# Peter00796/dlrover_wuqiong

Measured on AMD Instinct MI355X. Metric: ckpt save/load sec GPT2-1.5B; goodput% under injected faults at 1/2/4/8 GPU, lower is better.
Workload: dtype bf16

## Files before the change

dlrover_wuqiong_amd/_native/kernel_sigs.py:

```python

import ctypes as c

vp, i64, i32, u32, u64, f32, cp = (c.c_void_p, c.c_int64, c.c_int, c.c_uint32, c.c_uint64,
                                   c.c_float, c.c_char_p)

SIGS = {
    "dw_fp8_cast_amax": (i32, [vp, i32, vp, vp, vp, i64, i32, vp]),
    "dw_fp8_update_scales": (i32, [vp, vp, vp, vp, vp, i32, i32, i32, f32, vp]),
    "dw_fp8_cast_t": (i32, [vp, i32, vp, vp, vp, vp, i32, i32, i32, vp]),
    "dw_multi_copy": (i32, [vp, i64, vp]),
    "dw_gemm_dgelu": (i32, [vp, vp, vp, vp, i32, i32, i32, vp]),
    "dw_gemm_dgelu_bgrad": (i32, [vp, vp, vp, vp, vp, i32, i32, i32, vp]),
    "dw_gemm_wgrad_bgradb": (i32, [vp, vp, vp, vp, i32, i32, i32, i32, vp]),
    "dw_multi_copy_grid": (i32, [vp, i64, i32, vp]),
    "dw_multi_copy_variant": (i32, [vp, i64, i32, i32, vp]),
    "dw_fill_u32": (i32, [vp, i64, u32, vp]),
    "dw_host_register": (i32, [vp, u64]),
    "dw_host_unregister": (i32, [vp]),
    "dw_host_registered": (i32, [vp]),
    "dw_memcpy_async": (i32, [vp, vp, u64, i32, vp]),
    "dw_stream_sync": (i32, [vp]),
    "dw_event_sync": (i32, [vp]),
    "dw_stream_create_cumask": (vp, [i32, c.POINTER(i32)]),
    "dw_stream_destroy": (i32, [vp]),
# ... 39 lines not shown
    "dw_norm_fwd": (i32, [vp, vp, vp, vp, vp, vp, i64, i32, f32, i32, vp]),
    "dw_bias_gelu_fwd": (i32, [vp, vp, vp, vp, i64, i32, vp]),
    "dw_gelu_bwd": (i32, [vp, vp, vp, i64, vp]),
    "dw_colsum_parts": (i32, [i64]),
    "dw_colsum": (i32, [vp, i64, i32, vp, vp, i32, vp]),
    "dw_qadamw": (i32, [vp, vp, vp, vp, vp, vp, i64, i64, i32, i32, i32, f32, f32, f32, f32, f32, f32, f32, f32,
                        vp]),
    "dw_qadam_flat": (i32, [vp, i32, vp, vp, i32, vp, vp, vp, vp, vp, i64, i64, f32, f32, f32, f32, f32, f32, f32,
                            i32, vp, i32, vp]),
    "dw_colsum_acc": (i32, [vp, i64, i32, vp, vp, i32, i32, vp, vp]),
    "dw_gelu_bwd_dbias": (i32, [vp, vp, vp, i64, i32, vp, vp, i32, i32, vp, vp]),
    "dw_norm_bwd": (i32, [vp, vp, vp, vp, vp, vp, vp, vp, vp, vp, vp, i64, i64, i32, i32, i32, i32, vp, vp, vp]),
    "dw_norm_bwd_part_floats": (i64, [i64, i32, i32]),
    "dw_colred_det_floats": (i64, [i64, i32, i32]),
    "dw_add_norm_fwd": (i32, [vp, vp, vp, vp, vp, vp, vp, vp, i64, i32, f32, i32, vp]),
    "dw_swiglu_fwd": (i32, [vp, vp, i64, i32, vp]),
    "dw_swiglu_bwd": (i32, [vp, vp, vp, i64, i32, vp]),
    "dw_rope": (i32, [vp, vp, vp, vp, i64, i32, i32, i32, i32, vp, i32, vp]),
    "dw_qkv_rope": (i32, [vp, vp, vp, vp, vp, vp, i64, i32, i32, i32, i32, i32, vp, i32, vp]),
    "dw_grouped_gemm": (i32, [i32, vp, vp, vp, vp, i32, i32, i32, i32, i32, c.c_longlong, c.c_longlong,
                              c.c_longlong, c.c_longlong, c.c_longlong, vp]),
    "dw_grouped_glu_fwd": (i32, [vp, vp, vp, vp, vp, vp, i32, i32, i32, i32, vp]),
    "dw_grouped_glu_dgrad": (i32, [vp, vp, vp, vp, vp, i32, i32, i32, i32, vp]),
    "dw_xent_fwd": (i32, [vp, vp, vp, vp, vp, vp, i64, i32, i64, i64, f32, vp]),
    "dw_xent_bwd": (i32, [vp, vp, vp, vp, i32, vp, i64, i32, i64, i64, f32, vp]),
    "dw_token_logprob_fwd": (i32, [vp, i32, vp, vp, vp, vp, i64, i64, i64, i64, i32, vp]),
    "dw_token_logprob_bwd": (i32, [vp, i32, vp, vp, vp, vp, vp, vp, i64, i64, i64, i64, i32, vp]),
    "dw_sample_tokens": (i32, [vp, i32, vp, vp, i32, i32, i64, f32, i32, f32, u64, vp]),
    "dw_kv_append_rope": (i32, [vp, vp, vp, vp, vp, vp, vp, i64, i32, i32, i32, i32, i32, i64, i64, i32, vp]),
    "dw_rollout_step": (i32, [vp, vp, vp, vp, vp, vp, vp, i32, i64, i64, i64, vp]),
    "dw_moe_route_ws_floats": (i64, [i64]),
    "dw_moe_route_fwd": (i32, [vp, i32, vp, vp, vp, vp, vp, vp, vp, i64, i32, i32, i32, f32, f32, vp]),
    "dw_moe_route_bwd": (i32, [vp, i32, vp, vp, vp, vp, vp, vp, vp, i64, i32, i32, i32, f32, f32, vp]),
    "dw_moe_sort_ws_size": (i64, [i64, i32]),
    "dw_moe_sort_chunk_size": (i32, []),
    "dw_moe_sort": (i32, [vp, i64, i32, vp, vp, vp, vp, vp]),
    "dw_moe_gather_rows": (i32, [vp, vp, vp, vp, vp, vp, vp, i32, i64, i64, i32, i32, vp]),
    "dw_moe_ksum_rows": (i32, [vp, vp, vp, vp, vp, i32, i64, i64, i32, i32, vp]),
}

class AttnExtArgs(c.Structure):

    _fields_ = [("bias_bs", i64), ("bias_hs", i64), ("bias_qs", i64), ("bias", vp), ("prefix", vp), ("seed", u64),
                ("offset", u64), ("win_l", i32), ("win_r", i32), ("p_drop", f32), ("pad_", i32), ("alibi", vp),
                ("alibi_bs", i64)]


class AttnCall(c.Structure):

    _fields_ = [("q", vp), ("k", vp), ("v", vp), ("o", vp), ("lse", vp), ("dout", vp), ("dq", vp), ("dk", vp),
                ("dv", vp), ("workspace", vp), ("strides", i64 * 16), ("cu_q", vp), ("cu_k", vp),
                ("ext", AttnExtArgs), ("stream", vp), ("B", i32), ("Sq", i32), ("Sk", i32), ("H", i32),
                ("HKV", i32), ("D", i32), ("total_q", i32), ("total_k", i32), ("causal", i32), ("variant", i32),
                ("softmax_scale", f32), ("pad_", i32)]


OPTIONAL = {
    "dw_attn_fwd": (i32, [c.POINTER(AttnCall)]),
    "dw_attn_bwd": (i32, [c.POINTER(AttnCall)]),
    "dw_attn_bwd_workspace": (i64, [i32, i32, i32, i32]),
    "dw_attn_call_size": (i32, []),
    "dw_attn_dropout_mask": (i32, [vp, i32, i32, i32, f32, u64, u64, vp]),
    "dw_attn_decode": (i32, [vp, vp, vp, vp, vp, vp, vp, i32, i32, i32, i32, i32, i32, vp, f32, vp]),
    "dw_moe_regroup": (i32, [vp, vp, vp, i32, i32, i64, i32, i32, vp]),
}


def declare(lib):
    for name, (res, args) in SIGS.items():
        f = getattr(lib, name)
        f.restype = res
        f.argtypes = args
    for name, (res, args) in OPTIONAL.items():
        f = getattr(lib, name, None)
        if f is not None:
            f.restype = res
            f.argtypes = args
    size = getattr(lib, "dw_attn_call_size", None)
    if size is not None and size() != c.sizeof(AttnCall):
        raise RuntimeError(f"AttnCall ABI mismatch: library {size()} bytes, ctypes mirror {c.sizeof(AttnCall)}")
```

dlrover_wuqiong_amd/csrc/kernels/attn_bwd.hip:

```cpp
#include "attn_common.h"

#include <cstdlib>

typedef __attribute__((ext_vector_type(4))) short s16x4;
typedef __attribute__((address_space(3))) s16x4 lds_s16x4;
#define LDS_PTR(p) ((__attribute__((address_space(3))) void*)(p))

__device__ __forceinline__ bf16x8_t as_bf(const u32x4& v) { return __builtin_bit_cast(bf16x8_t, v); }

__device__ __forceinline__ unsigned int pk2(float a, float b) {
  typedef __bf16 bf16x2_v __attribute__((ext_vector_type(2)));
  typedef float f32x2_v __attribute__((ext_vector_type(2)));
  return __builtin_bit_cast(unsigned int, __builtin_convertvector((f32x2_v){a, b}, bf16x2_v));
}

__device__ __forceinline__ u32x4 scaled8(const u32x4& v, float c) {
  float f[8];
  unpack8(v, f);
  return (u32x4){pk2(f[0] * c, f[1] * c), pk2(f[2] * c, f[3] * c), pk2(f[4] * c, f[5] * c), pk2(f[6] * c, f[7] * c)};
}

template <int D>
__device__ __forceinline__ u32x4 tr_frag(const char* img, int r0, int d0, const int (&tr)[2]) {
  const s16x4 v0 =
      __builtin_amdgcn_ds_read_tr16_b64_v4i16((lds_s16x4*)LDS_PTR(img + tr[0] + tr_const<D>(r0, d0 / 32, 0)));
  const s16x4 v1 =
      __builtin_amdgcn_ds_read_tr16_b64_v4i16((lds_s16x4*)LDS_PTR(img + tr[1] + tr_const<D>(r0, d0 / 32, 1)));
  return join_tr(v0, v1);
}

template <int D>
__global__ void __launch_bounds__(256) attn_bwd_pre_kernel(const bf16_t* __restrict__ O, const bf16_t* __restrict__ dO,
                                                           float* __restrict__ delta, int B, int S, int H,
                                                           AttnStrides st) {
  constexpr int LPR = D / 8;
  constexpr int RPW = 64 / LPR;
  const int lane = threadIdx.x & 63;
  const int64_t row = ((int64_t)blockIdx.x * 4 + (threadIdx.x >> 6)) * RPW + lane / LPR;
  const int c = lane % LPR;
  const bool ok = row < (int64_t)B * S * H;
  float acc = 0.f;
  int h = 0, s = 0, b = 0;
  if (ok) {
    h = (int)(row % H);
    const int64_t bs = row / H;
    s = (int)(bs % S);
    b = (int)(bs / S);
    float a[8], d[8];
    unpack8(*(const u32x4*)(O + (int64_t)b * st.o_bs + (int64_t)s * st.o_rs + h * D + c * 8), a);
    unpack8(*(const u32x4*)(dO + (int64_t)b * st.do_bs + (int64_t)s * st.do_rs + h * D + c * 8), d);
#pragma unroll
    for (int k = 0; k < 8; ++k) acc += a[k] * d[k];
  }
#pragma unroll
  for (int off = LPR / 2; off > 0; off >>= 1) acc += __shfl_xor(acc, off, 64);
  if (ok && c == 0) delta[((int64_t)b * H + h) * S + s] = acc;
}


template <int D>
struct DkvCfg {
  static constexpr int WAVES = 4;
  static constexpr int BKB = 32 * WAVES;
  static constexpr int BQT = D == 64 ? 64 : 32;
  static constexpr int NCH = D / 8;
  static constexpr int KK = D / 16;
  static constexpr int DT = D / 32;
  static constexpr int TILE = BQT * D * 2;
  static constexpr int BUF = 2 * TILE + 2 * BQT * 4;
  static constexpr int VPT = BQT * NCH / (64 * WAVES);
  static constexpr int VIMG = BKB * D * 2;
};

template <int D, bool CAUSAL, bool PARTIAL, bool EXT>
__global__ void __launch_bounds__(64 * DkvCfg<D>::WAVES, (D == 64 && !EXT) ? 3 : 2)
attn_bwd_dkdv_kernel(const bf16_t* __restrict__ Q, const bf16_t* __restrict__ K, const bf16_t* __restrict__ V,
                     const bf16_t* __restrict__ dO, const float* __restrict__ LSE, const float* __restrict__ DELTA,
                     bf16_t* __restrict__ dK, bf16_t* __restrict__ dV, float* __restrict__ dKp,
                     float* __restrict__ dVp, int S, int H, int HKV, float scale, float scale_log2,
                     AttnStrides st, AttnVarlen vl, AttnExt ex) {
  using C = DkvCfg<D>;
  extern __shared__ __attribute__((aligned(16))) char smem[];
  const int tid = threadIdx.x, lane = tid & 63;
  const int wid = __builtin_amdgcn_readfirstlane(tid >> 6);
  const int r = lane & 31, hh = lane >> 5;
  const BlockXYZ bc = xcd_block((S + C::BKB - 1) / C::BKB, H);
  const int b = bc.z, h = bc.y;
  const int hk = h / (H / HKV);
  const int kb0 = bc.x * C::BKB;
  const SeqRange sr = seq_range(vl, b, h, H, S);
  if (kb0 >= sr.sk) return;
  const int SQ = sr.sq, SK = sr.sk, co = SK - SQ;
  const int kw0 = kb0 + 32 * wid;
  const int key = kw0 + r;
  const bf16_t* Qb = Q + (int64_t)b * st.q_bs + (int64_t)sr.q_off * st.q_rs + (int64_t)h * D;
  const bf16_t* dOb = dO + (int64_t)b * st.do_bs + (int64_t)sr.q_off * st.do_rs + (int64_t)h * D;
  const bf16_t* Kb = K + (int64_t)b * st.k_bs + (int64_t)sr.k_off * st.k_rs + (int64_t)hk * D;
  const bf16_t* Vb = V + (int64_t)b * st.v_bs + (int64_t)sr.k_off * st.v_rs + (int64_t)hk * D;
  const float* lse_b = LSE + sr.lse_base;
  const float* del_b = DELTA + sr.lse_base;

  char* v_img = smem + 2 * C::BUF;
  constexpr bool VDMA = !EXT && (C::VIMG / 1024) % C::WAVES == 0;
  if constexpr (VDMA) {
    constexpr int NGV = C::VIMG / 1024 / C::WAVES;
#pragma unroll
    for (int j = 0; j < NGV; ++j) {
      const int ci = NGV * wid + j;
      int row, ch;
      dma_rc<D>(ci, lane, row, ch);
      const int kv = min(kb0 + row, SK - 1);
      __builtin_amdgcn_global_load_lds((const void*)(Vb + (int64_t)kv * st.v_rs + ch * 8),
                                       LDS_PTR(v_img + 1024 * ci), 16, 0, 0);
    }
  }
  for (int v = tid; v < (VDMA ? 0 : C::BKB * C::NCH); v += 64 * C::WAVES) {
    int row, c;
    stage_rc<D>(v, row, c);
    const int kv = kb0 + row;
    *(u32x4*)(v_img + img_off<D>(row, c)) =
        kv < SK ? *(const u32x4*)(Vb + (int64_t)kv * st.v_rs + c * 8) : (u32x4){0, 0, 0, 0};
  }
  u32x4 kf[C::KK];
#pragma unroll
  for (int kk = 0; kk < C::KK; ++kk)
    kf[kk] = key < SK ? scaled8(*(const u32x4*)(Kb + (int64_t)key * st.k_rs + 16 * kk + 8 * hh), scale_log2)
                      : (u32x4){0, 0, 0, 0};
  f32x16 dk[C::DT], dv[C::DT];
#pragma unroll
  for (int dt = 0; dt < C::DT; ++dt)
#pragma unroll
    for (int i = 0; i < 16; ++i) {
      dk[dt][i] = 0.f;
// ... 144 lines not shown
          for (int j = 0; j < 4; ++j) {
            const int i = 4 * g + j;
            {
              const int q = q0 + qi + j;
              const bool vis = (q < SQ) && ext_visible(ex, CAUSAL, q, key, co, SK, pre);
              float add = (vis && ex.bias)
                  ? ex.bias[(int64_t)b * ex.bias_bs + (int64_t)h * ex.bias_hs + (int64_t)q * ex.bias_qs + key] *
                        1.4426950408889634f
                  : 0.f;
              add -= al2 * fabsf((float)(key - q - co));
              const float p = vis ? __builtin_amdgcn_exp2f(s[i] + add) : 0.f;
              if (ex.dropout) {
                const float del = -stl[C::BQT + qi + j];
                const bool kp = attn_keep(ex, bh, (long long)sr.q_off + q, (long long)sr.k_off + key);
                s[i] = kp ? p * ex.inv_keep : 0.f;
                dp[i] = p * (kp ? (dp[i] + del) * ex.inv_keep - del : -del);
              } else {
                s[i] = p;
                dp[i] = p * dp[i];
              }
            }
          }
        }
#pragma unroll
        for (int s2 = 0; s2 < 2; ++s2) {
          const u32x4 pf = {pk2(s[8 * s2 + 0], s[8 * s2 + 1]), pk2(s[8 * s2 + 2], s[8 * s2 + 3]),
                            pk2(s[8 * s2 + 4], s[8 * s2 + 5]), pk2(s[8 * s2 + 6], s[8 * s2 + 7])};
          const u32x4 sf = {pk2(dp[8 * s2 + 0], dp[8 * s2 + 1]), pk2(dp[8 * s2 + 2], dp[8 * s2 + 3]),
                            pk2(dp[8 * s2 + 4], dp[8 * s2 + 5]), pk2(dp[8 * s2 + 6], dp[8 * s2 + 7])};
#pragma unroll
          for (int dt = 0; dt < C::DT; ++dt) {
            const u32x4 doT = tr_frag<D>(dl, 32 * qs + 16 * s2, 32 * dt, trl);
            dv[dt] = __builtin_amdgcn_mfma_f32_32x32x16_bf16(as_bf(doT), as_bf(pf), dv[dt], 0, 0, 0);
          }
#pragma unroll
          for (int dt = 0; dt < C::DT; ++dt) {
            const u32x4 qT = tr_frag<D>(ql, 32 * qs + 16 * s2, 32 * dt, trl);
            dk[dt] = __builtin_amdgcn_mfma_f32_32x32x16_bf16(as_bf(qT), as_bf(sf), dk[dt], 0, 0, 0);
          }
        }
      }
    }
    if (it + 1 < n_it) {
      write((it + 1) & 1);
      if (!DMA && it + 2 < n_it) issue(it + 2);
    }
    if constexpr (DMA) asm volatile("s_waitcnt vmcnt(0)" ::: "memory");
    __syncthreads();
    if (DMA && it + 2 < n_it) {
      dma(it + 2, it & 1);
      issue(it + 2);
    }
  }
  if (key >= SK) return;
  if (PARTIAL) {
    const int64_t prow = vl.cu_q ? (int64_t)sr.k_off + key : (int64_t)b * S + key;
    float* kp = dKp + (prow * H + h) * D;
    float* vp = dVp + (prow * H + h) * D;
#pragma unroll
    for (int dt = 0; dt < C::DT; ++dt)
#pragma unroll
      for (int g = 0; g < 4; ++g) {
        const int d = 32 * dt + 8 * g + 4 * hh;
        *(f32x4*)(kp + d) = (f32x4){dk[dt][4 * g] * scale, dk[dt][4 * g + 1] * scale, dk[dt][4 * g + 2] * scale,
                                    dk[dt][4 * g + 3] * scale};
        *(f32x4*)(vp + d) = (f32x4){dv[dt][4 * g], dv[dt][4 * g + 1], dv[dt][4 * g + 2], dv[dt][4 * g + 3]};
      }
  } else {
    bf16_t* dKk = dK + (int64_t)b * st.dk_bs + (int64_t)hk * D + (int64_t)(sr.k_off + key) * st.dk_rs;
    bf16_t* dVk = dV + (int64_t)b * st.dv_bs + (int64_t)hk * D + (int64_t)(sr.k_off + key) * st.dv_rs;
#pragma unroll
    for (int dt = 0; dt < C::DT; ++dt)
#pragma unroll
      for (int g = 0; g < 4; ++g) {
        const int d = 32 * dt + 8 * g + 4 * hh;
        uint2 wk, wv;
        wk.x = pk2(dk[dt][4 * g] * scale, dk[dt][4 * g + 1] * scale);
        wk.y = pk2(dk[dt][4 * g + 2] * scale, dk[dt][4 * g + 3] * scale);
        wv.x = pk2(dv[dt][4 * g], dv[dt][4 * g + 1]);
        wv.y = pk2(dv[dt][4 * g + 2], dv[dt][4 * g + 3]);
        *(uint2*)(dKk + d) = wk;
        *(uint2*)(dVk + d) = wv;
      }
  }
}

template <int D>
__global__ void gqa_reduce_kernel(const float* __restrict__ pk, const float* __restrict__ pv, bf16_t* __restrict__ dK,
                                  bf16_t* __restrict__ dV, int64_t BS, int S, int H, int HKV, AttnStrides st) {
  const int group = H / HKV;
  const int64_t nv = BS * HKV * (D / 8);
  for (int64_t i = blockIdx.x * (int64_t)blockDim.x + threadIdx.x; i < nv; i += (int64_t)gridDim.x * blockDim.x) {
    const int c = (int)(i % (D / 8));
    const int64_t t = i / (D / 8);
    const int hk = (int)(t % HKV);
    const int64_t bs = t / HKV;
    const int64_t b = bs / S, sq = bs % S;
    float fk[8] = {0, 0, 0, 0, 0, 0, 0, 0}, fv[8] = {0, 0, 0, 0, 0, 0, 0, 0};
    for (int g = 0; g < group; ++g) {
      const int64_t off = (bs * H + hk * group + g) * D + c * 8;
      const f32x4 a0 = *(const f32x4*)(pk + off), a1 = *(const f32x4*)(pk + off + 4);
      const f32x4 b0 = *(const f32x4*)(pv + off), b1 = *(const f32x4*)(pv + off + 4);
#pragma unroll
      for (int j = 0; j < 4; ++j) {
        fk[j] += a0[j];
        fk[4 + j] += a1[j];
        fv[j] += b0[j];
        fv[4 + j] += b1[j];
      }
    }
    *(u32x4*)(dK + b * st.dk_bs + sq * st.dk_rs + hk * D + c * 8) = pack8(fk);
    *(u32x4*)(dV + b * st.dv_bs + sq * st.dv_rs + hk * D + c * 8) = pack8(fv);
  }
}

template <int D>
struct DqCfg {
  static constexpr int WAVES = D == 64 ? 4 : 8;
  static constexpr int BQ = 32 * WAVES;
  static constexpr int BK = 64;
  static constexpr int NCH = D / 8;
  static constexpr int KK = D / 16;
  static constexpr int DT = D / 32;
  static constexpr int TILE = BK * D * 2;
  static constexpr int VPT = BK * NCH / (64 * WAVES);
};

template <int D, bool CAUSAL, bool EXT>
__global__ void __launch_bounds__(64 * DqCfg<D>::WAVES, (D == 64 && !EXT) ? 3 : 1)
attn_bwd_dq_kernel(const bf16_t* __restrict__ Q, const bf16_t* __restrict__ K, const bf16_t* __restrict__ V,
                   const bf16_t* __restrict__ dO, const float* __restrict__ LSE, const float* __restrict__ DELTA,
                   bf16_t* __restrict__ dQ, int S, int H, int HKV, float scale, float scale_log2, AttnStrides st,
                   AttnVarlen vl, AttnExt ex) {
  using C = DqCfg<D>;
  extern __shared__ __attribute__((aligned(16))) char smem[];
  const int tid = threadIdx.x, lane = tid & 63;
  const int wid = __builtin_amdgcn_readfirstlane(tid >> 6);
  const int r = lane & 31, hh = lane >> 5;
  const int nqb = (S + C::BQ - 1) / C::BQ;
  const BlockXYZ bc = xcd_block(nqb, H);
  const int b = bc.z, h = bc.y;
  const int hk = h / (H / HKV);
  const int qblk = CAUSAL ? nqb - 1 - bc.x : bc.x;
  const int q_blk0 = qblk * C::BQ;
  const SeqRange sr = seq_range(vl, b, h, H, S);
  if (q_blk0 >= sr.sq) return;
  const int SQ = sr.sq, SK = sr.sk, co = SK - SQ;
  const int q0 = q_blk0 + wid * 32;
  const int q = q0 + r;
  const bf16_t* Qb = Q + (int64_t)b * st.q_bs + (int64_t)sr.q_off * st.q_rs + (int64_t)h * D;
  const bf16_t* dOb = dO + (int64_t)b * st.do_bs + (int64_t)sr.q_off * st.do_rs + (int64_t)h * D;
  const bf16_t* Kb = K + (int64_t)b * st.k_bs + (int64_t)sr.k_off * st.k_rs + (int64_t)hk * D;
  const bf16_t* Vb = V + (int64_t)b * st.v_bs + (int64_t)sr.k_off * st.v_rs + (int64_t)hk * D;

  constexpr bool RI = !EXT && D == 128;
  u32x4 qf[C::KK], dof[C::KK];
#pragma unroll
  for (int kk = 0; kk < C::KK; ++kk) {
    if (q < SQ) {
      qf[kk] = *(const u32x4*)(Qb + (int64_t)q * st.q_rs + 16 * kk + 8 * hh);
      if (RI) qf[kk] = scaled8(qf[kk], scale_log2);
      dof[kk] = *(const u32x4*)(dOb + (int64_t)q * st.do_rs + 16 * kk + 8 * hh);
    } else {
      qf[kk] = (u32x4){0, 0, 0, 0};
      dof[kk] = (u32x4){0, 0, 0, 0};
    }
  }
  const int64_t so = sr.lse_base + q;
  const float lse_v = q < SQ ? LSE[so] : -INFINITY;
  const float lse2 = lse_v > -INFINITY ? lse_v * 1.4426950408889634f : INFINITY;
  const float dl = q < SQ ? DELTA[so] : 0.f;

  f32x16 acc[C::DT];
#pragma unroll
  for (int dt = 0; dt < C::DT; ++dt)
#pragma unroll
    for (int i = 0; i < 16; ++i) acc[dt][i] = 0.f;
  constexpr bool DPI = !EXT && D == 64;
  f32x16 s_init, dp_init;
#pragma unroll
  for (int i = 0; i < 16; ++i) {
    s_init[i] = -lse2;
    dp_init[i] = -dl;
  }

  int n_tiles = (SK + C::BK - 1) / C::BK;
// ... 111 lines not shown
        if (!EXT) {
          if (need_mask) {
            __asm__ volatile("");
            const int rel = lim - k0 - 32 * sb - 4 * hh;
#pragma unroll
            for (int i = 0; i < 16; ++i) s[i] = ((i & 3) + 8 * (i >> 2)) < rel ? s[i] : -INFINITY;
          }
#pragma unroll
          for (int i = 0; i < 16; ++i) {
            if (RI) {
              s[i] = __builtin_amdgcn_exp2f(s[i]) * dp[i];
            } else {
              const float p = __builtin_amdgcn_exp2f(__builtin_fmaf(s[i], scale_log2, -lse2));
              s[i] = p * (DPI ? dp[i] : dp[i] - dl);
            }
          }
        }
#pragma unroll
        for (int i = 0; i < 16 && EXT; ++i) {
          {
            const int key = k0 + 32 * sb + (i & 3) + 8 * (i >> 2) + 4 * hh;
            const bool vis = (q < SQ) && ext_visible(ex, CAUSAL, q, key, co, SK, pre);
            float add = (vis && brow) ? brow[key] * 1.4426950408889634f : 0.f;
            add -= al2 * fabsf((float)(key - q - co));
            const float p = vis ? __builtin_amdgcn_exp2f(__builtin_fmaf(s[i], scale_log2, add - lse2)) : 0.f;
            float dpe = dp[i];
            if (ex.dropout)
              dpe = attn_keep(ex, bh, (long long)sr.q_off + q, (long long)sr.k_off + key) ? dpe * ex.inv_keep : 0.f;
            s[i] = p * (dpe - dl);
          }
        }
#pragma unroll
        for (int s2 = 0; s2 < 2; ++s2) {
          const u32x4 pf = {pk2(s[8 * s2 + 0], s[8 * s2 + 1]), pk2(s[8 * s2 + 2], s[8 * s2 + 3]),
                            pk2(s[8 * s2 + 4], s[8 * s2 + 5]), pk2(s[8 * s2 + 6], s[8 * s2 + 7])};
#pragma unroll
          for (int dt = 0; dt < C::DT; ++dt) {
            const u32x4 kt = tr_frag<D>(kl, 32 * sb + 16 * s2, 32 * dt, trl);
            acc[dt] = __builtin_amdgcn_mfma_f32_32x32x16_bf16(as_bf(kt), as_bf(pf), acc[dt], 0, 0, 0);
          }
        }
      }
      };
      tile();
    }
    if (!DMA && tt + 1 < n_run) {
      write_lds((tt + 1) & 1);
      if (tt + 2 < n_run) issue_load(t + 2);
    }
    if constexpr (DMA) asm volatile("s_waitcnt vmcnt(0)" ::: "memory");
    __syncthreads();
    if (DMA && tt + 2 < n_run) dma(t + 2, tt & 1);
  }
  if (q < SQ) {
    bf16_t* dQq = dQ + (int64_t)b * st.dq_bs + (int64_t)h * D + (int64_t)(sr.q_off + q) * st.dq_rs;
#pragma unroll
    for (int dt = 0; dt < C::DT; ++dt)
#pragma unroll
      for (int g = 0; g < 4; ++g) {
        uint2 w;
        w.x = pk2(acc[dt][4 * g + 0] * scale, acc[dt][4 * g + 1] * scale);
        w.y = pk2(acc[dt][4 * g + 2] * scale, acc[dt][4 * g + 3] * scale);
        *(uint2*)(dQq + 32 * dt + 8 * g + 4 * hh) = w;
      }
  }
}

extern "C" int64_t dw_attn_bwd_workspace(int B, int S, int H, int D) {
  return (int64_t)B * H * S * 4 + 2 * (int64_t)B * S * H * D * 4 + 512;
}

struct SideStream {
  hipStream_t s = nullptr;
  hipEvent_t fork = nullptr, join = nullptr;
};

static SideStream* side_stream() {
  static thread_local SideStream per_dev[16];
  int d = 0;
  if (hipGetDevice(&d) != hipSuccess || d < 0 || d >= 16) return nullptr;
  SideStream& ss = per_dev[d];
  if (!ss.s) {
    if (hipStreamCreateWithFlags(&ss.s, hipStreamNonBlocking) != hipSuccess) return nullptr;
    if (hipEventCreateWithFlags(&ss.fork, hipEventDisableTiming) != hipSuccess ||
        hipEventCreateWithFlags(&ss.join, hipEventDisableTiming) != hipSuccess)
      return nullptr;
  }
  return &ss;
}

static bool bwd_concurrent() {
  static const bool on = [] {
    const char* v = getenv("DWAMD_ATTN_BWD_CONCURRENT");
    return !(v && v[0] == '0');
  }();
  return on;
}

template <int D>
static void launch_bwd(const AttnCall& c, const AttnVarlen& vl, const AttnExt* ext) {
  const AttnExt none = {};
  const AttnExt& ex = ext ? *ext : none;
  const AttnStrides& st = c.st;
  const int B = c.B, Sq = c.Sq, Sk = c.Sk, H = c.H, HKV = c.HKV;
  const bool causal = c.causal;
  hipStream_t s = (hipStream_t)c.stream;
  char* ws = (char*)c.workspace;
  const bf16_t *q = (const bf16_t*)c.q, *k = (const bf16_t*)c.k, *v = (const bf16_t*)c.v;
  const bf16_t* dout = (const bf16_t*)c.dout;
  const float* lse = (const float*)c.lse;
  const int Smax = Sq > Sk ? Sq : Sk;
  float* delta = (float*)ws;
  const int pre_b = vl.cu_q ? 1 : B, pre_s = vl.cu_q ? vl.total_q : Sq;
  const int64_t rows = (int64_t)pre_b * pre_s * H;
  constexpr int RPB = 4 * (64 / (D / 8));
  hipLaunchKernelGGL(attn_bwd_pre_kernel<D>, dim3((unsigned)((rows + RPB - 1) / RPB)), dim3(256), 0, s,
                     (const bf16_t*)c.o, dout, delta, pre_b, pre_s, H, st);
  const float scale_log2 = c.softmax_scale * 1.4426950408889634f;
  SideStream* side = bwd_concurrent() ? side_stream() : nullptr;
  hipStream_t sq = s;
  if (side && hipEventRecord(side->fork, s) == hipSuccess && hipStreamWaitEvent(side->s, side->fork, 0) == hipSuccess)
    sq = side->s;
  using KC = DkvCfg<D>;
  const bool partial = H != HKV;
  float* pk = (float*)(ws + (((int64_t)B * H * Smax * 4 + 255) / 256) * 256);
  float* pv = pk + (int64_t)B * Smax * H * D;
  dim3 gk((unsigned)((Sk + KC::BKB - 1) / KC::BKB * H * B));
  const int lk = 2 * KC::BUF + KC::VIMG;
#define DKDV(CA, PA, EX)                                                                                    \
  hipLaunchKernelGGL((attn_bwd_dkdv_kernel<D, CA, PA, EX>), gk, dim3(64 * KC::WAVES), lk, s, q, k, v, dout, \
                     lse, delta, (bf16_t*)c.dk, (bf16_t*)c.dv, pk, pv, Sk, H, HKV, c.softmax_scale,         \
                     scale_log2, st, vl, ex)
  if (ext) {
    if (causal) {
      if (partial) DKDV(true, true, true); else DKDV(true, false, true);
    } else {
      if (partial) DKDV(false, true, true); else DKDV(false, false, true);
    }
  } else if (causal) {
    if (partial) DKDV(true, true, false); else DKDV(true, false, false);
  } else {
    if (partial) DKDV(false, true, false); else DKDV(false, false, false);
  }
#undef DKDV
  if (partial) {
    const int64_t prow = vl.cu_q ? (int64_t)vl.total_k : (int64_t)B * Sk;
    const int pS = vl.cu_q ? vl.total_k : Sk;
    const int64_t nv = prow * HKV * (D / 8);
    hipLaunchKernelGGL(gqa_reduce_kernel<D>, dim3(dw_grid_for(nv, 256, 4096)), dim3(256), 0, s, pk, pv,
                       (bf16_t*)c.dk, (bf16_t*)c.dv, prow, pS, H, HKV, st);
  }
  using DC = DqCfg<D>;
  dim3 gq((unsigned)((Sq + DC::BQ - 1) / DC::BQ * H * B));
  const int lq = 4 * DC::TILE;
#define DQ(CA, EX)                                                                                             \
  hipLaunchKernelGGL((attn_bwd_dq_kernel<D, CA, EX>), gq, dim3(64 * DC::WAVES), lq, sq, q, k, v, dout, lse,    \
                     delta, (bf16_t*)c.dq, Sq, H, HKV, c.softmax_scale, scale_log2, st, vl, ex)
  if (ext) {
    if (causal) DQ(true, true); else DQ(false, true);
  } else if (causal) {
    DQ(true, false);
  } else {
    DQ(false, false);
  }
#undef DQ
  if (sq != s) {
    (void)hipEventRecord(side->join, sq);
    (void)hipStreamWaitEvent(s, side->join, 0);
  }
}

extern "C" int dw_attn_bwd(const AttnCall* c) {
  if (!c || !attn_call_valid(*c)) return (int)hipErrorInvalidValue;
  const AttnVarlen vl = call_varlen(*c);
  const AttnExt ex = call_ext(*c);
  const AttnExt* ep = ext_active(&c->ext) ? &ex : nullptr;
  if (c->D == 128) launch_bwd<128>(*c, vl, ep);
  else launch_bwd<64>(*c, vl, ep);
  DW_LAUNCH_RET;
}

DW_PRELOAD(attn_bwd_pre_kernel<128>);
```

dlrover_wuqiong_amd/csrc/kernels/attn_common.h:

```cpp
#pragma once
#include "dw_common.h"

typedef __attribute__((ext_vector_type(16))) float f32x16;

template <int D>
__device__ __forceinline__ int img_off(int row, int ch) {
  return (D * 16) * (row >> 3) + 512 * (ch >> 2) + 64 * (row & 7) + 16 * ((ch & 3) ^ ((row >> 2) & 3));
}

template <int D>
__device__ __forceinline__ int row_lane(int lane, int kodd) {
  const int r = lane & 31, hh = lane >> 5;
  return (D * 16) * (r >> 3) + 64 * (r & 7) + 16 * ((2 * kodd + hh) ^ ((r >> 2) & 3));
}

template <int D>
__host__ __device__ constexpr int row_const(int row0, int kk) {
  return (D * 16) * (row0 >> 3) + 512 * (kk >> 1);
}

template <int D>
__device__ __forceinline__ int tr_lane(int lane, int p8) {
  const int hh = lane >> 5, g4 = lane >> 4, tq = (lane & 15) >> 2, tp = lane & 3;
  return 64 * (4 * hh + tq) + 16 * ((2 * (g4 & 1) + (tp >> 1)) ^ ((hh + 2 * p8) & 3)) + 8 * (tp & 1);
// ... 108 lines not shown
  long long tq, tk;
  unsigned int drop_thresh;
  float inv_keep;
  int win_l, win_r;
  bool dropout;
};

static inline AttnExt make_ext(const AttnExtArgs* a, long long tq, long long tk) {
  AttnExt e = {};
  e.win_l = e.win_r = -1;
  e.inv_keep = 1.f;
  if (!a) return e;
  e.bias = a->bias;
  e.bias_bs = a->bias_bs;
  e.bias_hs = a->bias_hs;
  e.bias_qs = a->bias_qs;
  e.prefix = a->prefix;
  e.alibi = a->alibi;
  e.alibi_bs = a->alibi_bs;
  e.seed = a->seed;
  e.offset = a->offset;
  e.tq = tq;
  e.tk = tk;
  e.win_l = a->win_l;
  e.win_r = a->win_r;
  e.dropout = a->p_drop > 0.f;
  if (e.dropout) {
    const double t = (double)a->p_drop * 4294967296.0;
    e.drop_thresh = t >= 4294967295.0 ? 0xFFFFFFFFu : (unsigned int)t;
    e.inv_keep = 1.f / (1.f - a->p_drop);
  }
  return e;
}

static inline bool ext_active(const AttnExtArgs* a) {
  return a && (a->bias || a->prefix || a->alibi || a->win_l >= 0 || a->win_r >= 0 || a->p_drop > 0.f);
}

struct AttnCall {
  const void *q, *k, *v;
  void *o, *lse;
  const void* dout;
  void *dq, *dk, *dv, *workspace;
  AttnStrides st;
  const int *cu_q, *cu_k;
  AttnExtArgs ext;
  void* stream;
  int B, Sq, Sk, H, HKV, D;
  int total_q, total_k;
  int causal;
  int variant;
  float softmax_scale;
  int pad_;
};

static inline bool attn_call_valid(const AttnCall& c) {
  if (c.HKV <= 0 || c.H % c.HKV != 0 || (c.D != 64 && c.D != 128) || !c.cu_q != !c.cu_k) return false;
  if (c.cu_q) return !(c.ext.bias || c.ext.prefix || (c.ext.alibi && c.ext.alibi_bs));
  return c.Sq == c.Sk;
}

static inline AttnVarlen call_varlen(const AttnCall& c) { return {c.cu_q, c.cu_k, c.total_q, c.total_k}; }

static inline AttnExt call_ext(const AttnCall& c) {
  return c.cu_q ? make_ext(&c.ext, c.total_q, c.total_k) : make_ext(&c.ext, c.Sq, c.Sk);
}

__device__ __forceinline__ unsigned int attn_hash(unsigned long long seed, unsigned long long idx) {
  unsigned long long z = seed + (idx + 1ull) * 0x9E3779B97F4A7C15ull;
  z = (z ^ (z >> 30)) * 0xBF58476D1CE4E5B9ull;
  z = (z ^ (z >> 27)) * 0x94D049BB133111EBull;
  return (unsigned int)((z ^ (z >> 31)) >> 32);
}

__device__ __forceinline__ bool attn_keep(const AttnExt& e, long long bh, long long qg, long long kg) {
  const unsigned long long idx = ((unsigned long long)bh * e.tq + qg) * e.tk + kg + e.offset;
  return attn_hash(e.seed, idx) >= e.drop_thresh;
}

__device__ __forceinline__ bool ext_visible(const AttnExt& e, bool causal, int q, int key, int co, int SK, int pre) {
  if (key >= SK) return false;
  if (key < pre) return true;
  const int d = key - (q + co);
  bool v = !causal || d <= 0;
  if (e.win_r >= 0) v = v && d <= e.win_r;
  if (e.win_l >= 0) v = v && d >= -e.win_l;
  return v;
}

__device__ __forceinline__ float ext_alibi2(const AttnExt& e, int b, int h) {
  return e.alibi ? e.alibi[(long long)b * e.alibi_bs + h] * 1.4426950408889634f : 0.f;
}
```

dlrover_wuqiong_amd/ops/attention.py:

```python

import ctypes
import math

import torch
import torch.nn.functional as F

from . import _hip
from .._native.kernel_sigs import AttnCall, AttnExtArgs


def _dense_hd(t: torch.Tensor) -> torch.Tensor:
    return t if (t.stride(3) == 1 and t.stride(2) == t.shape[3]) else t.contiguous()


def _rows_dense(t: torch.Tensor) -> torch.Tensor:
    return t if (t.stride(2) == 1 and t.stride(1) == t.shape[2]) else t.contiguous()


def _new_seed() -> int:
    return int(torch.randint(0, 2 ** 62, (1,), dtype=torch.int64).item())


_NO_EXT = ((-1, -1), None, None, None, 0.0, 0)
_Strides = ctypes.c_int64 * 16


def _attn_call(q, k, v, o, lse, causal, scale, ext, cu, bwd=()) -> AttnCall:
    ts = (q, k, v, o) + tuple(bwd)
    st = []
    if cu is None:
        D = q.shape[3]
        for t in ts:
            s = t.stride()
            assert s[3] == 1 and s[2] == D, "head/dim must be dense"
            st += s[:2]
        B, Sq, Sk, tq, tk, cu_q, cu_k = q.shape[0], q.shape[1], q.shape[1], 0, 0, None, None
    else:
        for t in ts:
            st += (0, t.stride(0))
        B, Sq, Sk, tq, tk = cu[0].numel() - 1, int(cu[2]), int(cu[3]), q.shape[0], k.shape[0]
        cu_q, cu_k = cu[0].data_ptr(), cu[1].data_ptr()
    return AttnCall(*[t.data_ptr() for t in ts[:4]], lse.data_ptr(), *[t.data_ptr() for t in ts[4:]] or (None,) * 4,
                    None, _Strides(*st), cu_q, cu_k, _ext_args(ext), torch.cuda.current_stream().cuda_stream, B, Sq,
                    Sk, q.shape[-2], k.shape[-2], q.shape[-1], tq, tk, int(causal), 0, float(scale))


def _ext_args(ext) -> AttnExtArgs:
    if ext is _NO_EXT:
        return _NO_EXT_ARGS
    window, bias, prefix, alibi, p_drop, seed = ext
    a = AttnExtArgs(win_l=int(window[0]), win_r=int(window[1]), p_drop=float(p_drop), seed=int(seed) & ((1 << 64) - 1))
    if bias is not None:
        a.bias = bias.data_ptr()
        a.bias_bs, a.bias_hs, a.bias_qs = bias.stride(0), bias.stride(1), bias.stride(2)
    if prefix is not None:
        a.prefix = prefix.data_ptr()
    if alibi is not None:
        a.alibi = alibi.data_ptr()
        a.alibi_bs = alibi.stride(0) if alibi.dim() == 2 else 0
    return a


_NO_EXT_ARGS = AttnExtArgs(win_l=-1, win_r=-1)


def _attn_fwd(q, k, v, causal, scale, ext=_NO_EXT, cu=None):
    H = q.shape[-2]
    o = torch.empty(q.shape, device=q.device, dtype=q.dtype)
    lse = torch.empty((q.shape[0], H, q.shape[1]) if cu is None else (H, q.shape[0]), device=q.device,
                      dtype=torch.float32)
    c = _attn_call(q, k, v, o, lse, causal, scale, ext, cu)
    _hip.check(_hip.lib().dw_attn_fwd(ctypes.byref(c)), "attn_fwd")
    return o, lse


def _attn_bwd(q, k, v, o, lse, do, causal, scale, ext=_NO_EXT, cu=None, grads=None):
    dq, dk, dv = grads if grads is not None else (torch.empty_like(q), torch.empty_like(k), torch.empty_like(v))
    c = _attn_call(q, k, v, o, lse, causal, scale, ext, cu, (do, dq, dk, dv))
    L = _hip.lib()
    ws = torch.empty(L.dw_attn_bwd_workspace(c.B, max(c.Sq, c.Sk), c.H, c.D), device=q.device, dtype=torch.uint8)
    c.workspace = ws.data_ptr()
    _hip.check(L.dw_attn_bwd(ctypes.byref(c)), "attn_bwd")
    return dq, dk, dv


class _FlashAttnQKVPackedFn(torch.autograd.Function):

    @staticmethod
    def forward(ctx, qkv, causal, scale):
        _hip.require_bf16(qkv)
        B, S, _three, H, D = qkv.shape
        if qkv.stride(4) != 1 or qkv.stride(3) != D or qkv.stride(2) != H * D:
            qkv = qkv.contiguous()
        o, lse = _attn_fwd(*qkv.unbind(2), causal, scale)
        ctx.save_for_backward(qkv, o, lse)
        ctx.causal, ctx.scale = causal, scale
        return o

    @staticmethod
    def backward(ctx, do):
        qkv, o, lse = ctx.saved_tensors
        do = _dense_hd(do.to(torch.bfloat16))
        dqkv = torch.empty_like(qkv)
        _attn_bwd(*qkv.unbind(2), o, lse, do, ctx.causal, ctx.scale, grads=dqkv.unbind(2))
        return dqkv, None, None


def flash_attn_qkvpacked_func(qkv, causal: bool = True, softmax_scale=None):
    D = qkv.shape[-1]
    scale = softmax_scale if softmax_scale is not None else 1.0 / math.sqrt(D)
    if _hip.bf16_path(qkv):
        return _FlashAttnQKVPackedFn.apply(_hip.bf16(qkv), causal, scale)
    q, k, v = qkv.unbind(2)
    return flash_attn_func(q, k, v, softmax_scale=scale, causal=causal)


class _FlashAttnFn(torch.autograd.Function):

    @staticmethod
    def forward(ctx, q, k, v, causal, scale, ext=None):
        _hip.require_bf16(q, k, v)
        q, k, v = _dense_hd(q), _dense_hd(k), _dense_hd(v)
        window, bias, prefix, alibi, p_drop, seed = ext or _NO_EXT
        o, lse = _attn_fwd(q, k, v, causal, scale, ext or _NO_EXT)
        ctx.save_for_backward(q, k, v, o, lse, bias, prefix, alibi)
        ctx.meta = (causal, scale, tuple(window), p_drop, seed, ext is None)
        if ext is None:
            return o
        ctx.mark_non_differentiable(lse)
        return o, lse

    @staticmethod
    def backward(ctx, do, _dlse=None):
        q, k, v, o, lse, bias, prefix, alibi = ctx.saved_tensors
        causal, scale, window, p_drop, seed, plain = ctx.meta
        do = _dense_hd(do.to(torch.bfloat16))
        ext = _NO_EXT if plain else (window, bias, prefix, alibi, p_drop, seed)
        dq, dk, dv = _attn_bwd(q, k, v, o, lse, do, causal, scale, ext)
        return dq, dk, dv, None, None, None


def attention_reference(q, k, v, causal=True, softmax_scale=None):
    B, S, H, D = q.shape
    HKV = k.shape[2]
    scale = softmax_scale if softmax_scale is not None else 1.0 / math.sqrt(D)
    qf, kf, vf = q.float().transpose(1, 2), k.float().transpose(1, 2), v.float().transpose(1, 2)
    if HKV != H:
        kf = kf.repeat_interleave(H // HKV, dim=1)
        vf = vf.repeat_interleave(H // HKV, dim=1)
    s = torch.matmul(qf, kf.transpose(-1, -2)) * scale
    if causal:
        mask = torch.ones(S, S, dtype=torch.bool, device=q.device).triu(1)
        s = s.masked_fill(mask, float("-inf"))
    p = torch.softmax(s, dim=-1)
    o = torch.matmul(p, vf)
    return o.transpose(1, 2).to(q.dtype)




def _prep_bias(bias, B, H, Sq, Sk, device):
    if bias is None:
        return None
    if bias.dtype == torch.bool:
        bias = torch.zeros(bias.shape, dtype=torch.float32, device=bias.device).masked_fill_(~bias, float("-inf"))
# ... 312 lines not shown
```

Before: 0.009400.

## Fold QKV bias gradient reduction into flash attention backward kernels

```diff
diff --git a/dlrover_wuqiong_amd/_native/kernel_sigs.py b/dlrover_wuqiong_amd/_native/kernel_sigs.py
--- a/dlrover_wuqiong_amd/_native/kernel_sigs.py
+++ b/dlrover_wuqiong_amd/_native/kernel_sigs.py
@@ -115,7 +115,8 @@
                 ("dv", vp), ("workspace", vp), ("strides", i64 * 16), ("cu_q", vp), ("cu_k", vp),
                 ("ext", AttnExtArgs), ("stream", vp), ("B", i32), ("Sq", i32), ("Sk", i32), ("H", i32),
                 ("HKV", i32), ("D", i32), ("total_q", i32), ("total_k", i32), ("causal", i32), ("variant", i32),
-                ("softmax_scale", f32), ("pad_", i32)]
+                ("softmax_scale", f32), ("pad_", i32), ("dbias_ws", vp), ("dbias", vp), ("dbias_fp32", i32),
+                ("dbias_acc", i32)]
 
 
 OPTIONAL = {
diff --git a/dlrover_wuqiong_amd/csrc/kernels/attn_bwd.hip b/dlrover_wuqiong_amd/csrc/kernels/attn_bwd.hip
--- a/dlrover_wuqiong_amd/csrc/kernels/attn_bwd.hip
+++ b/dlrover_wuqiong_amd/csrc/kernels/attn_bwd.hip
@@ -27,6 +27,58 @@
   const s16x4 v1 =
       __builtin_amdgcn_ds_read_tr16_b64_v4i16((lds_s16x4*)LDS_PTR(img + tr[1] + tr_const<D>(r0, d0 / 32, 1)));
   return join_tr(v0, v1);
+}
+
+struct BiasFold {
+  float* ws;
+  void* out;
+  int out_fp32, accumulate;
+};
+
+constexpr int FOLD_TILE = 32 * 64 * 4;
+
+__device__ __forceinline__ void fold_put(char* reg, const f32x16 (&a)[2], int r, int hh) {
+#pragma unroll
+  for (int dt = 0; dt < 2; ++dt)
+#pragma unroll
+    for (int g = 0; g < 4; ++g) {
+      const int c = 8 * dt + 2 * g + hh;
+      *(f32x4*)(reg + 256 * r + 16 * (c ^ (r & 15))) =
+          (f32x4){a[dt][4 * g], a[dt][4 * g + 1], a[dt][4 * g + 2], a[dt][4 * g + 3]};
+    }
+}
+
+__device__ __forceinline__ float fold_get(const char* reg, int lane) {
+  float s[4] = {0.f, 0.f, 0.f, 0.f};
+#pragma unroll
+  for (int r = 0; r < 32; ++r)
+    s[r & 3] += *(const float*)(reg + 256 * r + 16 * ((lane >> 2) ^ (r & 15)) + 4 * (lane & 3));
+  return (s[0] + s[1]) + (s[2] + s[3]);
+}
+
+__device__ __forceinline__ void fold_finish(const BiasFold& bf, int n_cols, int slot, unsigned n_wg, int lane, int c0,
+                                            int c1) {
+  asm volatile("s_waitcnt vmcnt(0)" ::: "memory");
+  unsigned* cnt = (unsigned*)(bf.ws + n_cols) + slot;
+  unsigned prev = 0;
+  if (lane == 0) prev = __hip_atomic_fetch_add(cnt, 1u, __ATOMIC_RELAXED, __HIP_MEMORY_SCOPE_AGENT);
+  if ((unsigned)__builtin_amdgcn_readfirstlane((int)prev) != n_wg - 1) return;
+  float v[2];
+  v[0] = __hip_atomic_exchange(bf.ws + c0 + lane, 0.f, __ATOMIC_RELAXED, __HIP_MEMORY_SCOPE_AGENT);
+  if (c1 >= 0) v[1] = __hip_atomic_exchange(bf.ws + c1 + lane, 0.f, __ATOMIC_RELAXED, __HIP_MEMORY_SCOPE_AGENT);
+#pragma unroll
+  for (int k = 0; k < 2; ++k) {
+    if (k == 1 && c1 < 0) break;
+    const int c = (k ? c1 : c0) + lane;
+    if (bf.out_fp32) {
+      float* o = (float*)bf.out;
+      o[c] = bf.accumulate ? o[c] + v[k] : v[k];
+    } else {
+      bf16_t* o = (bf16_t*)bf.out;
+      o[c] = f2bf(bf.accumulate ? bf2f(o[c]) + v[k] : v[k]);
+    }
+  }
+  if (lane == 0) __hip_atomic_exchange(cnt, 0u, __ATOMIC_RELAXED, __HIP_MEMORY_SCOPE_AGENT);
 }
 
 template <int D>
@@ -78,7 +130,7 @@
                      const bf16_t* __restrict__ dO, const float* __restrict__ LSE, const float* __restrict__ DELTA,
                      bf16_t* __restrict__ dK, bf16_t* __restrict__ dV, float* __restrict__ dKp,
                      float* __restrict__ dVp, int S, int H, int HKV, float scale, float scale_log2,
-                     AttnStrides st, AttnVarlen vl, AttnExt ex) {
+                     AttnStrides st, AttnVarlen vl, AttnExt ex, BiasFold bf) {
   using C = DkvCfg<D>;
   extern __shared__ __attribute__((aligned(16))) char smem[];
   const int tid = threadIdx.x, lane = tid & 63;
@@ -329,8 +381,36 @@
       issue(it + 2);
     }
   }
-  if (key >= SK) return;
-  if (PARTIAL) {
+  if constexpr (D == 64 && !PARTIAL && !EXT) {
+    if (bf.ws) {
+      static_assert(C::WAVES * FOLD_TILE + 2 * C::WAVES * 256 <= 2 * C::BUF + C::VIMG, "fold tiles fit the LDS");
+      char* reg = smem + wid * FOLD_TILE;
+      float* comb = (float*)(smem + C::WAVES * FOLD_TILE);
+      fold_put(reg, dk, r, hh);
+      __syncthreads();
+      const float sk_ = fold_get(reg, lane);
+      __syncthreads();
+      fold_put(reg, dv, r, hh);
+      __syncthreads();
+      const float sv_ = fold_get(reg, lane);
+      comb[wid * 64 + lane] = sk_ * scale;
+      comb[(C::WAVES + wid) * 64 + lane] = sv_;
+      __syncthreads();
+      if (wid == 0) {
+        const int HD = H * D;
+        float tk = 0.f, tv = 0.f;
+#pragma unroll
+        for (int w = 0; w < C::WAVES; ++w) {
+          tk += comb[w * 64 + lane];
+          tv += comb[(C::WAVES + w) * 64 + lane];
+        }
+        atomicAdd(bf.ws + HD + h * D + lane, tk);
+        atomicAdd(bf.ws + 2 * HD + h * D + lane, tv);
+      }
+    }
+  }
+  if (key >= SK) {
+  } else if (PARTIAL) {
     const int64_t prow = vl.cu_q ? (int64_t)sr.k_off + key : (int64_t)b * S + key;
     float* kp = dKp + (prow * H + h) * D;
     float* vp = dVp + (prow * H + h) * D;
@@ -359,6 +439,10 @@
         *(uint2*)(dKk + d) = wk;
         *(uint2*)(dVk + d) = wv;
       }
+  }
+  if constexpr (D == 64 && !PARTIAL && !EXT) {
+    if (bf.ws && wid == 0)
+      fold_finish(bf, 3 * H * D, H + h, gridDim.x / H, lane, (H + h) * D, (2 * H + h) * D);
   }
 }
 
@@ -408,7 +492,7 @@
 attn_bwd_dq_kernel(const bf16_t* __restrict__ Q, const bf16_t* __restrict__ K, const bf16_t* __restrict__ V,
                    const bf16_t* __restrict__ dO, const float* __restrict__ LSE, const float* __restrict__ DELTA,
                    bf16_t* __restrict__ dQ, int S, int H, int HKV, float scale, float scale_log2, AttnStrides st,
-                   AttnVarlen vl, AttnExt ex) {
+                   AttnVarlen vl, AttnExt ex, BiasFold bf) {
   using C = DqCfg<D>;
   extern __shared__ __attribute__((aligned(16))) char smem[];
   const int tid = threadIdx.x, lane = tid & 63;
@@ -626,6 +710,25 @@
     __syncthreads();
     if (DMA && tt + 2 < n_run) dma(t + 2, tt & 1);
   }
+  if constexpr (D == 64 && !EXT) {
+    if (bf.ws) {
+      static_assert(C::WAVES * FOLD_TILE <= 4 * C::TILE, "fold tiles fit the LDS");
+      char* reg = smem + wid * FOLD_TILE;
+      fold_put(reg, acc, r, hh);
+      __syncthreads();
+      const float sq_ = fold_get(reg, lane);
+      __syncthreads();
+      float* comb = (float*)smem;
+      comb[wid * 64 + lane] = sq_ * scale;
+      __syncthreads();
+      if (wid == 0) {
+        float tq = 0.f;
+#pragma unroll
+        for (int w = 0; w < C::WAVES; ++w) tq += comb[w * 64 + lane];
+        atomicAdd(bf.ws + h * D + lane, tq);
+      }
+    }
+  }
   if (q < SQ) {
     bf16_t* dQq = dQ + (int64_t)b * st.dq_bs + (int64_t)h * D + (int64_t)(sr.q_off + q) * st.dq_rs;
 #pragma unroll
@@ -637,6 +740,10 @@
         w.y = pk2(acc[dt][4 * g + 2] * scale, acc[dt][4 * g + 3] * scale);
         *(uint2*)(dQq + 32 * dt + 8 * g + 4 * hh) = w;
       }
+  }
+  if constexpr (D == 64 && !EXT) {
+    if (bf.ws && wid == 0)
+      fold_finish(bf, 3 * H * D, h, gridDim.x / H, lane, h * D, -1);
   }
 }
 
@@ -683,6 +790,7 @@
   const bf16_t *q = (const bf16_t*)c.q, *k = (const bf16_t*)c.k, *v = (const bf16_t*)c.v;
   const bf16_t* dout = (const bf16_t*)c.dout;
   const float* lse = (const float*)c.lse;
+  const BiasFold bf = {(float*)c.dbias_ws, c.dbias, c.dbias_fp32, c.dbias_acc};
   const int Smax = Sq > Sk ? Sq : Sk;
   float* delta = (float*)ws;
   const int pre_b = vl.cu_q ? 1 : B, pre_s = vl.cu_q ? vl.total_q : Sq;
@@ -704,7 +812,7 @@
 #define DKDV(CA, PA, EX)                                                                                    \
   hipLaunchKernelGGL((attn_bwd_dkdv_kernel<D, CA, PA, EX>), gk, dim3(64 * KC::WAVES), lk, s, q, k, v, dout, \
                      lse, delta, (bf16_t*)c.dk, (bf16_t*)c.dv, pk, pv, Sk, H, HKV, c.softmax_scale,         \
-                     scale_log2, st, vl, ex)
+                     scale_log2, st, vl, ex, bf)
   if (ext) {
     if (causal) {
       if (partial) DKDV(true, true, true); else DKDV(true, false, true);
@@ -729,7 +837,7 @@
   const int lq = 4 * DC::TILE;
 #define DQ(CA, EX)                                                                                             \
   hipLaunchKernelGGL((attn_bwd_dq_kernel<D, CA, EX>), gq, dim3(64 * DC::WAVES), lq, sq, q, k, v, dout, lse,    \
-                     delta, (bf16_t*)c.dq, Sq, H, HKV, c.softmax_scale, scale_log2, st, vl, ex)
+                     delta, (bf16_t*)c.dq, Sq, H, HKV, c.softmax_scale, scale_log2, st, vl, ex, bf)
   if (ext) {
     if (causal) DQ(true, true); else DQ(false, true);
   } else if (causal) {
diff --git a/dlrover_wuqiong_amd/csrc/kernels/attn_common.h b/dlrover_wuqiong_amd/csrc/kernels/attn_common.h
--- a/dlrover_wuqiong_amd/csrc/kernels/attn_common.h
+++ b/dlrover_wuqiong_amd/csrc/kernels/attn_common.h
@@ -184,10 +184,13 @@
   int variant;
   float softmax_scale;
   int pad_;
+  void *dbias_ws, *dbias;
+  int dbias_fp32, dbias_acc;
 };
 
 static inline bool attn_call_valid(const AttnCall& c) {
   if (c.HKV <= 0 || c.H % c.HKV != 0 || (c.D != 64 && c.D != 128) || !c.cu_q != !c.cu_k) return false;
+  if (c.dbias_ws && (!c.dbias || c.D != 64 || c.cu_q || c.H != c.HKV || ext_active(&c.ext))) return false;
   if (c.cu_q) return !(c.ext.bias || c.ext.prefix || (c.ext.alibi && c.ext.alibi_bs));
   return c.Sq == c.Sk;
 }
diff --git a/dlrover_wuqiong_amd/ops/attention.py b/dlrover_wuqiong_amd/ops/attention.py
--- a/dlrover_wuqiong_amd/ops/attention.py
+++ b/dlrover_wuqiong_amd/ops/attention.py
@@ -1,12 +1,16 @@
 
 import ctypes
 import math
+import os
 
 import torch
 import torch.nn.functional as F
 
 from . import _hip
+from ._grad import claim, direct_grad, notify
 from .._native.kernel_sigs import AttnCall, AttnExtArgs
+
+_FOLD = os.environ.get("DWAMD_ATTN_FOLD_BIAS", "1") != "0"
 
 
 def _dense_hd(t: torch.Tensor) -> torch.Tensor:
@@ -74,10 +78,14 @@
     return o, lse
 
 
-def _attn_bwd(q, k, v, o, lse, do, causal, scale, ext=_NO_EXT, cu=None, grads=None):
+def _attn_bwd(q, k, v, o, lse, do, causal, scale, ext=_NO_EXT, cu=None, grads=None, dbias=None):
     dq, dk, dv = grads if grads is not None else (torch.empty_like(q), torch.empty_like(k), torch.empty_like(v))
     c = _attn_call(q, k, v, o, lse, causal, scale, ext, cu, (do, dq, dk, dv))
     L = _hip.lib()
+    if dbias is not None:
+        g, acc = dbias
+        c.dbias_ws = _hip.zeroed_workspace(g.numel() + 2 * c.H, q.device).data_ptr()
+        c.dbias, c.dbias_fp32, c.dbias_acc = g.data_ptr(), int(g.dtype == torch.float32), int(acc)
     ws = torch.empty(L.dw_attn_bwd_workspace(c.B, max(c.Sq, c.Sk), c.H, c.D), device=q.device, dtype=torch.uint8)
     c.workspace = ws.data_ptr()
     _hip.check(L.dw_attn_bwd(ctypes.byref(c)), "attn_bwd")
@@ -87,7 +95,8 @@
 class _FlashAttnQKVPackedFn(torch.autograd.Function):
 
     @staticmethod
-    def forward(ctx, qkv, causal, scale):
+    def forward(ctx, qkv, causal, scale, fold=None):
+        ctx.fold = fold
         _hip.require_bf16(qkv)
         B, S, _three, H, D = qkv.shape
         if qkv.stride(4) != 1 or qkv.stride(3) != D or qkv.stride(2) != H * D:
@@ -102,15 +111,39 @@
         qkv, o, lse = ctx.saved_tensors
         do = _dense_hd(do.to(torch.bfloat16))
         dqkv = torch.empty_like(qkv)
-        _attn_bwd(*qkv.unbind(2), o, lse, do, ctx.causal, ctx.scale, grads=dqkv.unbind(2))
-        return dqkv, None, None
+        fold, g = ctx.fold, None
+        if fold is not None and not _hip.deterministic():
+            g = direct_grad(fold[1])
+            if g is not None and (g.numel() != qkv.shape[2] * qkv.shape[3] * qkv.shape[4]
+                                  or g.dtype not in (torch.bfloat16, torch.float32)):
+                g = None
+        _attn_bwd(*qkv.unbind(2), o, lse, do, ctx.causal, ctx.scale, grads=dqkv.unbind(2),
+                  dbias=(g, not claim(fold[1])) if g is not None else None)
+        if g is not None:
+            fold[0].out_bias_folded = True
+            notify(fold[1])
+        return dqkv, None, None, None
+
+
+def _qkv_fold_target(qkv):
+    if not _FOLD or qkv.shape[-1] != 64:
+        return None
+    node = qkv.grad_fn
+    if node is not None and not hasattr(node, "out_bias") and node.name().startswith(("ViewBackward",
+                                                                                       "UnsafeViewBackward")):
+        node = node.next_functions[0][0]
+    b = getattr(node, "out_bias", None)
+    if b is None or direct_grad(b) is None or b.numel() != qkv.shape[2] * qkv.shape[3] * qkv.shape[4]:
+        return None
+    return (node, b)
 
 
 def flash_attn_qkvpacked_func(qkv, causal: bool = True, softmax_scale=None):
     D = qkv.shape[-1]
     scale = softmax_scale if softmax_scale is not None else 1.0 / math.sqrt(D)
     if _hip.bf16_path(qkv):
-        return _FlashAttnQKVPackedFn.apply(_hip.bf16(qkv), causal, scale)
+        qkv = _hip.bf16(qkv)
+        return _FlashAttnQKVPackedFn.apply(qkv, causal, scale, _qkv_fold_target(qkv))
     q, k, v = qkv.unbind(2)
     return flash_attn_func(q, k, v, softmax_scale=scale, causal=causal)
 
```

After: 0.01170. 1.24x slower.
